# zju-pi/diff-sampler

Measured on AMD Instinct MI355X. Metric: images/sec (whole node) at NFE=10, EDM CIFAR-10, higher is better.
Workload: dtype fp32; 1 GPU; EDM CIFAR-10 32x32 SongUNet (55.7M params), DPM-Solver++(2M) logSNR NFE=10, batch 256/GPU; launch=eager

## Files before the change

### diff_sampler_amd/csrc/conv3x3_wino.hip

```cpp
#include <type_traits>

#include "igemm_common.h"

namespace igemm {
namespace {

typedef float f32x2 __attribute__((ext_vector_type(2)));

constexpr int WV_NO_NORM = 2, WV_NO_HALO = 4, WV_NO_DMA = 8, WV_NO_EPI = 16;
constexpr int WINO_K = 8;
constexpr int WINO_POS = 2 * 64 * 4;
constexpr int WINO_IMG = 16 * WINO_POS;
constexpr int WINO_NSH = 4;
constexpr int WINO_EPI_LD = 36;

#define DS_WINO_WAIT_VM0() do { __builtin_amdgcn_s_waitcnt(0x0F70); asm volatile("" ::: "memory"); } while (0)
#define DS_WINO_WAIT_VM(n) do { __builtin_amdgcn_s_waitcnt(0x0F70 | (n)); asm volatile("" ::: "memory"); } while (0)

template <int VAR, int NORM, int NSL>
__global__ void __launch_bounds__(256, 1) conv3x3_wino_kernel(const KParams p) {
    extern __shared__ __attribute__((aligned(16))) float smem[];
    float* Us = smem;
    float* Vs = smem + 2 * WINO_IMG;
    float* Hs = Vs + WINO_IMG;

    const int tid = threadIdx.x, lane = tid & 63;
    const int wave = __builtin_amdgcn_readfirstlane(tid >> 6);
    const int wr = wave >> 1, wc = wave & 1;
    int mt, nt;
    if (!decode_tile(blockIdx.x, p.mtiles, p.ntiles, mt, nt)) return;
    const int m0 = mt * 256, n0 = nt * 64;
    const int img0 = m0 / p.HW;
    const int r0 = (m0 - img0 * p.HW) / p.W;
    const int WPH = p.WP >> 1, Wt = p.W >> 1;
    const int Ctot = p.c0 + p.c1;
    const int nslabs = Ctot / WINO_K;
    constexpr bool kDma = !(VAR & WV_NO_DMA), kHalo = !(VAR & WV_NO_HALO);
    constexpr int kNorm = (VAR & WV_NO_NORM) ? 0 : NORM;

    const int kh_h = tid & 1;
    unsigned h_off0[WINO_NSH], h_off1[WINO_NSH];
    int h_lds[WINO_NSH];
    bool h_ok[WINO_NSH];
#pragma unroll
    for (int j = 0; j < WINO_NSH; ++j) {
        const int hp = (tid + j * 256) >> 1;
        const int hr = hp / p.WP, hc = hp - hr * p.WP;
        const int y = r0 + hr - 1, x = hc - 1;
        const bool in = hp < p.NP;
        h_ok[j] = in && (unsigned)y < (unsigned)p.H && (unsigned)x < (unsigned)p.W;
        const int pix = min(max(y, 0), p.H - 1) * p.W + min(max(x, 0), p.W - 1);
        h_off0[j] = (unsigned)(pix * p.lda0 + kh_h * 4);
        h_off1[j] = (unsigned)(pix * p.lda1 + kh_h * 4);
        h_lds[j] = in ? (((kh_h * 2 + (hc & 1)) * p.HP + hr) * WPH + (hc >> 1)) * 4 : p.NP * WINO_K;
    }
    const float* a0i = p.a0 + (size_t)img0 * p.HW * p.lda0;
    const float* a1i = p.a1 + (size_t)img0 * p.HW * p.lda1;
    const float* cpi = p.norm + (size_t)img0 * 3 * Ctot + kh_h * 4;
    f32x4 hreg[WINO_NSH];
    float h_t[4 * WINO_NSH], h_u[4 * WINO_NSH];
    f32x4 cmu = {0.f, 0.f, 0.f, 0.f}, cga = {1.f, 1.f, 1.f, 1.f}, cbe = {0.f, 0.f, 0.f, 0.f};
    const float* h_src = nullptr;
    unsigned h_sel = 0;
    auto halo_src = [&](int s) {
        const int c = s * WINO_K;
        const bool first = c < p.c0;
        h_src = first ? a0i + c : a1i + (c - p.c0);
        h_sel = (unsigned)__builtin_amdgcn_readfirstlane(first ? -1 : 0);
        asm volatile("" : "+s"(h_sel));
    };
    auto halo_load1 = [&](auto J) {
        constexpr int j = decltype(J)::value;
        if constexpr (j >= NSL) return;
        const unsigned off = (h_off0[j] & h_sel) | (h_off1[j] & ~h_sel);
        hreg[j] = *reinterpret_cast<const f32x4*>(h_src + off);
    };
    auto coef_load1 = [&](int s, auto I) {
        constexpr int i = decltype(I)::value;
        if constexpr (NORM != 0) {
            const f32x4 v = *reinterpret_cast<const f32x4*>(cpi + (size_t)i * Ctot + s * WINO_K);
            if constexpr (i == 0) cmu = v; else if constexpr (i == 1) cga = v; else cbe = v;
        }
    };
    auto halo_chain = [&](auto C, auto ST) {
        constexpr int c = decltype(C)::value, st = decltype(ST)::value, j = c >> 2, e = c & 3;
        if constexpr (j >= NSL) return;
        if constexpr (st == 0 && kNorm != 0) {
            h_t[c] = __builtin_fmaf(hreg[j][e] - cmu[e], cga[e], cbe[e]);
            if constexpr (kNorm == 2) h_u[c] = __expf(-h_t[c]);
        }
        if constexpr (st == 1 && kNorm == 2) h_u[c] = __builtin_amdgcn_rcpf(1.0f + h_u[c]);
        if constexpr (st == 2) {
            float v = hreg[j][e];
            if constexpr (kNorm == 1) v = h_t[c];
            if constexpr (kNorm == 2) v = h_t[c] * h_u[c];
            hreg[j][e] = h_ok[j] ? v : 0.f;
            if constexpr (e == 3) *reinterpret_cast<f32x4*>(Hs + h_lds[j]) = hreg[j];
        }
    };

    const int t_t = (tid >> 1) & 63, cpl = tid & 1, kh_t = tid >> 7;
    const int t_ty = t_t / Wt, t_tx = t_t - t_ty * Wt;
    const float* h_rd = Hs + ((kh_t * 2 * p.HP + 2 * t_ty) * WPH + t_tx) * 4 + cpl * 2;
    const int h_par = p.HP * WPH * 4;
    float* v_wr = Vs + (kh_t * 64 + t_t) * 4 + cpl * 2;
    auto transform = [&]() {
        f32x2 d[4][4];
#pragma unroll
        for (int i = 0; i < 4; ++i)
#pragma unroll
            for (int j = 0; j < 4; ++j)
                d[i][j] = *reinterpret_cast<const f32x2*>(h_rd + (j & 1) * h_par + i * WPH * 4 + (j >> 1) * 4);
        DS_RACE_SKEW(wave);
        f32x2 t[4][4];
#pragma unroll
        for (int j = 0; j < 4; ++j) {
            t[0][j] = d[0][j] - d[2][j];
            t[1][j] = d[1][j] + d[2][j];
            t[2][j] = d[2][j] - d[1][j];
            t[3][j] = d[1][j] - d[3][j];
        }
#pragma unroll
        for (int i = 0; i < 4; ++i) {
            *reinterpret_cast<f32x2*>(v_wr + (i * 4 + 0) * WINO_POS) = t[i][0] - t[i][2];
            *reinterpret_cast<f32x2*>(v_wr + (i * 4 + 1) * WINO_POS) = t[i][1] + t[i][2];
            *reinterpret_cast<f32x2*>(v_wr + (i * 4 + 2) * WINO_POS) = t[i][2] - t[i][1];
            *reinterpret_cast<f32x2*>(v_wr + (i * 4 + 3) * WINO_POS) = t[i][1] - t[i][3];
        }
    };

    const float* u_src = p.b + (size_t)nt * nslabs * WINO_IMG + tid * 4;
    auto u_dma1 = [&](const float* src, float* ubuf, auto I) {
        constexpr int i = decltype(I)::value;
        float* dst = ubuf + (i * 256 + wave * 64) * 4;
        typedef const __attribute__((address_space(1))) void* gptr_t;
        typedef __attribute__((address_space(3))) void* lptr_t;
        __builtin_amdgcn_global_load_lds((gptr_t)(src + i * 1024), (lptr_t)(dst), 16, 0, 0);
    };

    f32x16 acc[16];
#pragma unroll
    for (int q = 0; q < 16; ++q)
#pragma unroll
        for (int r = 0; r < 16; ++r) acc[q][r] = 0.f;
    const int a_off = ((lane >> 5) * 64 + wr * 32 + (lane & 31)) * 4;
    const int b_off = ((lane >> 5) * 64 + wc * 32 + (lane & 31)) * 4;

#define DS_WINO_I(n) std::integral_constant<int, (n)>{}
#define DS_WINO_EACH4(F) F(0) F(1) F(2) F(3)
#define DS_WINO_EACH16(F, b) F((b) + 0) F((b) + 1) F((b) + 2) F((b) + 3) F((b) + 4) F((b) + 5) F((b) + 6) F((b) + 7)                \
                             F((b) + 8) F((b) + 9) F((b) + 10) F((b) + 11) F((b) + 12) F((b) + 13) F((b) + 14) F((b) + 15)

    halo_src(0);
#define DS_WINO_F(j) halo_load1(DS_WINO_I(j));
    DS_WINO_EACH4(DS_WINO_F)
#undef DS_WINO_F
    coef_load1(0, DS_WINO_I(0)); coef_load1(0, DS_WINO_I(1)); coef_load1(0, DS_WINO_I(2));
    DS_RACE_SKEW(wave);
#define DS_WINO_F(i) u_dma1(u_src, Us, DS_WINO_I(i)); u_dma1(u_src, Us, DS_WINO_I((i) + 4));
    DS_WINO_EACH4(DS_WINO_F)
#undef DS_WINO_F
    DS_RACE_SKEW(wave);
#define DS_WINO_F(c) halo_chain(DS_WINO_I(c), DS_WINO_I(0)); halo_chain(DS_WINO_I(c), DS_WINO_I(1)); halo_chain(DS_WINO_I(c), DS_WINO_I(2));
    DS_WINO_EACH16(DS_WINO_F, 0)
#undef DS_WINO_F
    {
        const int s1 = min(1, nslabs - 1);
        halo_src(s1);
#define DS_WINO_F(j) halo_load1(DS_WINO_I(j));
        DS_WINO_EACH4(DS_WINO_F)
#undef DS_WINO_F
        coef_load1(s1, DS_WINO_I(0)); coef_load1(s1, DS_WINO_I(1)); coef_load1(s1, DS_WINO_I(2));
    }
    DS_WINO_WAIT_VM0();
    __syncthreads();

    f32x4 fa[2][4], fb[2][4];
    int s = 0;
    do {
        const float* ub = Us + (s & 1) * WINO_IMG;
        transform();
        __syncthreads();
        const int s1 = min(s + 1, nslabs - 1), s2 = min(s + 2, nslabs - 1);
        const float* un = u_src + (size_t)s1 * WINO_IMG;
        float* ubn = Us + ((s + 1) & 1) * WINO_IMG;
        if constexpr (kHalo) halo_src(s2);
        auto frag_read = [&](auto G, auto I) {
            constexpr int g = decltype(G)::value, i = decltype(I)::value;
            if constexpr (i < 4) fa[g & 1][i] = *reinterpret_cast<const f32x4*>(Vs + (g * 4 + i) * WINO_POS + a_off);
            else fb[g & 1][i - 4] = *reinterpret_cast<const f32x4*>(ub + (g * 4 + i - 4) * WINO_POS + b_off);
        };
        if constexpr (kHalo) {
            DS_RACE_SKEW(wave);
#define DS_WINO_F(c) halo_chain(DS_WINO_I(c), DS_WINO_I(0)); halo_chain(DS_WINO_I(c), DS_WINO_I(1)); halo_chain(DS_WINO_I(c), DS_WINO_I(2));
            DS_WINO_EACH16(DS_WINO_F, 0)
#undef DS_WINO_F
        }
        auto fill = [&](auto K) {
            constexpr int k = decltype(K)::value, g = k >> 4;
            if constexpr (k < 8) {
                if constexpr (kDma) {
                    if constexpr (k == 0) DS_RACE_SKEW(wave);
                    u_dma1(un, ubn, DS_WINO_I(k));
                }
            } else if constexpr (k < 12) {
                if constexpr (kHalo) halo_load1(DS_WINO_I(k - 8));
            } else if constexpr (k < 15) {
                if constexpr (kHalo) coef_load1(s2, DS_WINO_I(k - 12));
            }
            constexpr int fr = g == 0 ? 8 : g == 1 ? 20 : g == 2 ? 32 : 64;
            if constexpr (k >= fr && k < fr + 8) frag_read(DS_WINO_I(g + 1), DS_WINO_I(k - fr));
        };
#define DS_WINO_STEP(k)                                                                                                                \
        acc[((k) >> 4) * 4 + ((k) & 3)] = __builtin_amdgcn_mfma_f32_32x32x2f32(fa[((k) >> 4) & 1][(k) & 3][((k) >> 2) & 3],            \
                                                                               fb[((k) >> 4) & 1][(k) & 3][((k) >> 2) & 3],            \
                                                                               acc[((k) >> 4) * 4 + ((k) & 3)], 0, 0, 0);              \
        fill(DS_WINO_I(k));                                                                                                            \
        __builtin_amdgcn_sched_barrier(0);
#define DS_WINO_F(i) frag_read(DS_WINO_I(0), DS_WINO_I(i)); frag_read(DS_WINO_I(0), DS_WINO_I((i) + 4));
        DS_WINO_EACH4(DS_WINO_F)
#undef DS_WINO_F
        __builtin_amdgcn_sched_barrier(0);
        DS_WINO_EACH16(DS_WINO_STEP, 0)
        DS_WINO_EACH16(DS_WINO_STEP, 16)
        DS_WINO_EACH16(DS_WINO_STEP, 32)
        DS_WINO_EACH16(DS_WINO_STEP, 48)
#undef DS_WINO_STEP
        DS_WINO_WAIT_VM0();
        __syncthreads();
    } while (++s < nslabs);

    if constexpr ((VAR & WV_NO_EPI) != 0) {
#pragma unroll
        for (int q = 0; q < 16; ++q) asm volatile("" :: "v"(acc[q]));
        return;
    }

    f32x16 Y[4];
#pragma unroll
    for (int a = 0; a < 2; ++a) {
        f32x16 t[4];
#pragma unroll
        for (int j = 0; j < 4; ++j) t[j] = a == 0 ? acc[j] + acc[4 + j] + acc[8 + j] : acc[4 + j] - acc[8 + j] - acc[12 + j];
        Y[a * 2 + 0] = t[0] + t[1] + t[2];
        Y[a * 2 + 1] = t[1] - t[2] - t[3];
    }

    const int nextra = (p.ec0 + p.ec1) / 32;
    if (nextra > 0) {
        const float* wsk = p.b + (size_t)p.ntiles * nslabs * WINO_IMG + (size_t)nt * nextra * 2048 + tid * 4;
        const int e_chunk = tid & 7;
        int e_lds[8];
#pragma unroll
        for (int j = 0; j < 8; ++j) {
            const int lp = (tid >> 3) + 32 * j;
            const int yl = lp / p.W, x = lp - yl * p.W;
            const int ph = (yl & 1) * 2 + (x & 1), t = (yl >> 1) * Wt + (x >> 1);
            e_lds[j] = (((ph * 4 + (e_chunk >> 1)) * 2 + (e_chunk & 1)) * 64 + (t ^ e_chunk)) * 4;
        }
        int ea_off[4];
#pragma unroll
        for (int g = 0; g < 4; ++g) ea_off[g] = ((lane >> 5) * 64 + ((wr * 32 + (lane & 31)) ^ (2 * g + (lane >> 5)))) * 4;
        const unsigned e_t0 = (unsigned)((tid >> 3) * p.elda0 + e_chunk * 4), e_t1 = (unsigned)((tid >> 3) * p.elda1 + e_chunk * 4);
        const float* e_src = nullptr;
        unsigned e_off = 0;
        int e_step = 0;
        auto e_sel = [&](int es) {
            const int c = es * 32;
            const bool first = c < p.ec0;
            const int ld = first ? p.elda0 : p.elda1;
            e_src = (first ? p.e0 + c : p.e1 + (c - p.ec0)) + (size_t)m0 * ld;
            e_step = 32 * ld;
            e_off = first ? e_t0 : e_t1;
        };
        auto e_load1 = [&](f32x4* dst, auto J) {
            constexpr int j = decltype(J)::value;
            dst[j] = *reinterpret_cast<const f32x4*>(e_src + (size_t)(j * e_step) + e_off);
        };
        auto w_dma1 = [&](int es, float* wbuf, auto I) {
            constexpr int i = decltype(I)::value;
            float* dst = wbuf + (i * 256 + wave * 64) * 4;
            typedef const __attribute__((address_space(1))) void* gptr_t;
            typedef __attribute__((address_space(3))) void* lptr_t;
            __builtin_amdgcn_global_load_lds((gptr_t)(wsk + (size_t)es * 2048 + i * 1024), (lptr_t)(dst), 16, 0, 0);
        };
#define DS_WINO_EACH8(F) F(0) F(1) F(2) F(3) F(4) F(5) F(6) F(7)

        f32x4 ereg[8];
        {
            f32x4 ereg0[8];
            DS_RACE_SKEW(wave);
            w_dma1(0, smem, DS_WINO_I(0)); w_dma1(0, smem, DS_WINO_I(1));
            e_sel(0);
#define DS_WINO_F(j) e_load1(ereg0, DS_WINO_I(j));
            DS_WINO_EACH8(DS_WINO_F)
#undef DS_WINO_F
            e_sel(min(1, nextra - 1));
#define DS_WINO_F(j) e_load1(ereg, DS_WINO_I(j));
            DS_WINO_EACH8(DS_WINO_F)
#undef DS_WINO_F
            DS_WINO_WAIT_VM(8);
            DS_RACE_SKEW(wave);
#pragma unroll
            for (int j = 0; j < 8; ++j) *reinterpret_cast<f32x4*>(Vs + e_lds[j]) = ereg0[j];
        }
        __syncthreads();

        f32x4 ga[2][4], gb[2];
        int es = 0;
        do {
            const float* vb = smem + (2 - (es & 1)) * WINO_IMG;
            float* vn = smem + (1 + (es & 1)) * WINO_IMG;
            const float* wb = smem + (es & 1) * 2048;
            float* wn = smem + ((es + 1) & 1) * 2048;
            const int es1 = min(es + 1, nextra - 1);
            e_sel(min(es + 2, nextra - 1));
            auto frag_read = [&](auto G, auto I) {
                constexpr int g = decltype(G)::value, i = decltype(I)::value;
                if constexpr (i < 4) ga[g & 1][i] = *reinterpret_cast<const f32x4*>(vb + (i * 4 + g) * WINO_POS + ea_off[g]);
                else gb[g & 1] = *reinterpret_cast<const f32x4*>(wb + g * WINO_POS + b_off);
            };
            auto fill = [&](auto K) {
                constexpr int k = decltype(K)::value, g = k >> 4;
                if constexpr (k < 2) {
                    if constexpr (k == 0) DS_RACE_SKEW(wave);
                    w_dma1(es1, wn, DS_WINO_I(k));
                } else if constexpr (k >= 7 && k < 15) {
                    if constexpr (k == 7) DS_RACE_SKEW(wave);
                    *reinterpret_cast<f32x4*>(vn + e_lds[k - 7]) = ereg[k - 7];
                } else if constexpr (k >= 15 && k < 23) {
                    e_load1(ereg, DS_WINO_I(k - 15));
                }
                constexpr int fr = g == 0 ? 2 : g == 1 ? 24 : g == 2 ? 36 : 64;
                if constexpr (k >= fr && k < fr + 5) frag_read(DS_WINO_I(g + 1), DS_WINO_I(k - fr));
            };
#define DS_WINO_STEP(k)                                                                                                                \
            Y[(k) & 3] = __builtin_amdgcn_mfma_f32_32x32x2f32(ga[((k) >> 4) & 1][(k) & 3][((k) >> 2) & 3], gb[((k) >> 4) & 1][((k) >> 2) & 3], \
                                                              Y[(k) & 3], 0, 0, 0);                                                    \
            fill(DS_WINO_I(k));                                                                                                        \
            __builtin_amdgcn_sched_barrier(0);
            frag_read(DS_WINO_I(0), DS_WINO_I(0)); frag_read(DS_WINO_I(0), DS_WINO_I(4)); frag_read(DS_WINO_I(0), DS_WINO_I(1));
            frag_read(DS_WINO_I(0), DS_WINO_I(2)); frag_read(DS_WINO_I(0), DS_WINO_I(3));
            __builtin_amdgcn_sched_barrier(0);
            DS_WINO_EACH16(DS_WINO_STEP, 0)
            DS_WINO_EACH16(DS_WINO_STEP, 16)
            DS_WINO_EACH16(DS_WINO_STEP, 32)
            DS_WINO_EACH16(DS_WINO_STEP, 48)
#undef DS_WINO_STEP
            DS_WINO_WAIT_VM0();
            __syncthreads();
        } while (++es < nextra);
#undef DS_WINO_EACH8
    }
#undef DS_WINO_EACH16
#undef DS_WINO_EACH4
#undef DS_WINO_I

    float* stage = smem + wave * 32 * WINO_EPI_LD;
    const int c4 = (lane & 7) * 4;
    const int col = n0 + wc * 32 + c4;
    f32x4 cb = {0.f, 0.f, 0.f, 0.f}, cvu = {0.f, 0.f, 0.f, 0.f};
    if (p.colbias) cb = *reinterpret_cast<const f32x4*>(p.colbias + col);
    if (p.cbias) cvu = *reinterpret_cast<const f32x4*>(p.cbias + (size_t)(p.cbias_bcast ? 0 : img0) * p.cbias_ld + col);
    const float acc_scale = __builtin_bit_cast(float, __builtin_amdgcn_readfirstlane(__builtin_bit_cast(int, p.acc_scale)));
    const float scale = __builtin_bit_cast(float, __builtin_amdgcn_readfirstlane(__builtin_bit_cast(int, p.scale)));
    int e_row[4];
#pragma unroll
    for (int pass = 0; pass < 4; ++pass) {
        const int tl = wr * 32 + pass * 8 + (lane >> 3);
        const int ty = tl / Wt, tx = tl - ty * Wt;
        e_row[pass] = m0 + 2 * ty * p.W + 2 * tx;
    }
#pragma unroll
    for (int a = 0; a < 2; ++a) {
        f32x4 st_s = {0.f, 0.f, 0.f, 0.f}, st_q = {0.f, 0.f, 0.f, 0.f};
#pragma unroll
        for (int b = 0; b < 2; ++b) {
            const f32x16 y = Y[a * 2 + b];
            f32x4 rv[4];
            if (p.res) {
#pragma unroll
                for (int pass = 0; pass < 4; ++pass)
                    rv[pass] = __builtin_nontemporal_load(reinterpret_cast<const f32x4*>(p.res + (size_t)(e_row[pass] + a * p.W + b) * p.res_ld + col));
            }
#pragma unroll
            for (int r = 0; r < 16; ++r) stage[((r & 3) + 8 * (r >> 2) + 4 * (lane >> 5)) * WINO_EPI_LD + (lane & 31)] = y[r];
#pragma unroll
            for (int pass = 0; pass < 4; ++pass) {
                f32x4 v = *reinterpret_cast<const f32x4*>(stage + (pass * 8 + (lane >> 3)) * WINO_EPI_LD + c4);
                v *= acc_scale;
                v += cb;
                if (p.cbias) v += cvu;
                if (p.res) v += rv[pass];
                v *= scale;
                if (p.act == DS_ACT_SILU) {
#pragma unroll
                    for (int q = 0; q < 4; ++q) v[q] = ds_silu(v[q]);
                }
                __builtin_nontemporal_store(v, reinterpret_cast<f32x4*>(p.out + (size_t)(e_row[pass] + a * p.W + b) * p.ldo + col));
                st_s += v; st_q += v * v;
            }
        }
        if (p.stats) {
#pragma unroll
            for (int q = 0; q < 4; ++q) {
                st_s[q] += __shfl_xor(st_s[q], 8); st_s[q] += __shfl_xor(st_s[q], 16); st_s[q] += __shfl_xor(st_s[q], 32);
                st_q[q] += __shfl_xor(st_q[q], 8); st_q[q] += __shfl_xor(st_q[q], 16); st_q[q] += __shfl_xor(st_q[q], 32);
            }
            if (lane < 8) {
                float* sp = p.stats + (size_t)((m0 >> 6) + wr * 2 + a) * 2 * p.N + col;
                *reinterpret_cast<f32x4*>(sp) = st_s;
                *reinterpret_cast<f32x4*>(sp + p.N) = st_q;
            }
        }
    }
}

template <int VAR, int NORM, int NSL>
int launch_wino_ns(KParams& p, hipStream_t stream) {
    const int smem = (3 * WINO_IMG + p.NP * WINO_K + 4) * (int)sizeof(float);
    DS_ENSURE_DYN_LDS((&conv3x3_wino_kernel<VAR, NORM, NSL>), 128 * 1024);
    hipLaunchKernelGGL((conv3x3_wino_kernel<VAR, NORM, NSL>), dim3(grid_1d(p.mtiles, p.ntiles)), dim3(256), smem, stream, p);
    DS_CHECK_LAUNCH();
    return DS_OK;
}

template <int VAR, int NORM>
int launch_wino_n(KParams& p, hipStream_t stream) {
    return p.NP * 2 <= 3 * 256 ? launch_wino_ns<VAR, NORM, 3>(p, stream) : launch_wino_ns<VAR, NORM, 4>(p, stream);
}

template <int VAR>
int launch_wino(KParams& p, hipStream_t stream) {
    if (!p.norm) return launch_wino_n<VAR, 0>(p, stream);
    return p.norm_act == DS_ACT_SILU ? launch_wino_n<VAR, 2>(p, stream) : launch_wino_n<VAR, 1>(p, stream);
}

}

bool conv3x3_wino_applicable(const KParams& p) {
    if (p.taps != 9 || p.stride != 1 || p.splits != 1 || (p.ec0 & 31) || (p.ec1 & 31)) return false;
    if ((p.H & 1) || (p.W & 1) || p.W < 4 || p.W > 64 || p.HW % 256 || 256 % p.W || ((256 / p.W) & 1)) return false;
    if ((p.N & 63) || (p.c0 % WINO_K) || (p.c1 % WINO_K) || !p.vec_ok || p.out_planar || p.out_f16 || p.res_f16 || p.rowbias) return false;
    if (p.act != DS_ACT_NONE && p.act != DS_ACT_SILU) return false;
    const int np = (256 / p.W + 2) * (p.W + 2);
    if (np * 2 > WINO_NSH * 256 || (3 * WINO_IMG + np * WINO_K + 4) * (int)sizeof(float) > 128 * 1024) return false;
    return p.M % 256 == 0;
}

int launch_conv3x3_wino(KParams& p, hipStream_t stream) {
    if (!conv3x3_wino_applicable(p)) return DS_E_SHAPE;
    p.TH = 256 / p.W; p.nimg = 1; p.HP = p.TH + 2; p.WP = p.W + 2; p.NP = p.HP * p.WP;
    p.mtiles = p.M / 256; p.ntiles = p.N / 64; p.n_begin = 0;
#ifdef DS_CONV_ABLATIONS
    if (p.t_variant & 0x10000) {
        switch (p.t_variant & 31) {
            case 2: return launch_wino<2>(p, stream);
            case 4: return launch_wino<4>(p, stream);
            case 8: return launch_wino<8>(p, stream);
            case 16: return launch_wino<16>(p, stream);
            case 28: return launch_wino<28>(p, stream);
            default: break;
        }
    }
#endif
    return launch_wino<0>(p, stream);
}

}
```

Before: 446.3 images/sec.

## Double-buffer Winograd V and halo LDS to drop per-slab barrier

Restructures the Winograd 3x3 conv main loop so the input transform for slab s+1 is computed into a second V buffer while the GEMM consumes slab s. The halo staging area is double-buffered, and halo loads are prefetched three slabs ahead using two register sets. This removes the mid-iteration __syncthreads and transform stall between transform and MMA. The cost is raising the LDS footprint to up to 160 KB, plus byte-offset address tricks meant to keep global loads in SGPR-base plus VGPR-offset form.

Result: faster. 463.6 images/sec (median of 6 runs) (+3.9%).

```diff
diff --git a/diff_sampler_amd/csrc/conv3x3_wino.hip b/diff_sampler_amd/csrc/conv3x3_wino.hip
--- a/diff_sampler_amd/csrc/conv3x3_wino.hip
+++ b/diff_sampler_amd/csrc/conv3x3_wino.hip
@@ -22,7 +22,7 @@
     extern __shared__ __attribute__((aligned(16))) float smem[];
     float* Us = smem;
     float* Vs = smem + 2 * WINO_IMG;
-    float* Hs = Vs + WINO_IMG;
+    float* Hs = smem + 4 * WINO_IMG;
 
     const int tid = threadIdx.x, lane = tid & 63;
     const int wave = __builtin_amdgcn_readfirstlane(tid >> 6);
@@ -50,16 +50,21 @@
         const bool in = hp < p.NP;
         h_ok[j] = in && (unsigned)y < (unsigned)p.H && (unsigned)x < (unsigned)p.W;
         const int pix = min(max(y, 0), p.H - 1) * p.W + min(max(x, 0), p.W - 1);
-        h_off0[j] = (unsigned)(pix * p.lda0 + kh_h * 4);
-        h_off1[j] = (unsigned)(pix * p.lda1 + kh_h * 4);
+        h_off0[j] = (unsigned)(pix * p.lda0 + kh_h * 4) * 4u;
+        h_off1[j] = (unsigned)(pix * p.lda1 + kh_h * 4) * 4u;
         h_lds[j] = in ? (((kh_h * 2 + (hc & 1)) * p.HP + hr) * WPH + (hc >> 1)) * 4 : p.NP * WINO_K;
     }
     const float* a0i = p.a0 + (size_t)img0 * p.HW * p.lda0;
     const float* a1i = p.a1 + (size_t)img0 * p.HW * p.lda1;
-    const float* cpi = p.norm + (size_t)img0 * 3 * Ctot + kh_h * 4;
-    f32x4 hreg[WINO_NSH];
+    const float* cpi = p.norm + (size_t)img0 * 3 * Ctot;
+    unsigned c_lane = (unsigned)(kh_h * 16);
+    const int h_buf = p.NP * WINO_K + 4;
+    struct HaloRegs {
+        f32x4 h[WINO_NSH];
+        f32x4 mu = {0.f, 0.f, 0.f, 0.f}, ga = {1.f, 1.f, 1.f, 1.f}, be = {0.f, 0.f, 0.f, 0.f};
+    };
+    HaloRegs hreg;
     float h_t[4 * WINO_NSH], h_u[4 * WINO_NSH];
-    f32x4 cmu = {0.f, 0.f, 0.f, 0.f}, cga = {1.f, 1.f, 1.f, 1.f}, cbe = {0.f, 0.f, 0.f, 0.f};
     const float* h_src = nullptr;
     unsigned h_sel = 0;
     auto halo_src = [&](int s) {
@@ -69,73 +74,70 @@
         h_sel = (unsigned)__builtin_amdgcn_readfirstlane(first ? -1 : 0);
         asm volatile("" : "+s"(h_sel));
     };
-    auto halo_load1 = [&](auto J) {
+    auto halo_load1 = [&](HaloRegs& R, auto J) {
         constexpr int j = decltype(J)::value;
         if constexpr (j >= NSL) return;
         const unsigned off = (h_off0[j] & h_sel) | (h_off1[j] & ~h_sel);
-        hreg[j] = *reinterpret_cast<const f32x4*>(h_src + off);
-    };
-    auto coef_load1 = [&](int s, auto I) {
+        R.h[j] = *reinterpret_cast<const f32x4*>(reinterpret_cast<const char*>(h_src) + off);
+    };
+    auto coef_load1 = [&](HaloRegs& R, int s, auto I) {
         constexpr int i = decltype(I)::value;
         if constexpr (NORM != 0) {
-            const f32x4 v = *reinterpret_cast<const f32x4*>(cpi + (size_t)i * Ctot + s * WINO_K);
-            if constexpr (i == 0) cmu = v; else if constexpr (i == 1) cga = v; else cbe = v;
-        }
-    };
-    auto halo_chain = [&](auto C, auto ST) {
+            const char* cs = reinterpret_cast<const char*>(cpi + (size_t)i * Ctot + s * WINO_K);
+            asm volatile("" : "+v"(c_lane));
+            const f32x4 v = *reinterpret_cast<const f32x4*>(cs + c_lane);
+            if constexpr (i == 0) R.mu = v; else if constexpr (i == 1) R.ga = v; else R.be = v;
+        }
+    };
+    auto halo_chain = [&](HaloRegs& R, float* hs, auto C, auto ST) {
         constexpr int c = decltype(C)::value, st = decltype(ST)::value, j = c >> 2, e = c & 3;
         if constexpr (j >= NSL) return;
         if constexpr (st == 0 && kNorm != 0) {
-            h_t[c] = __builtin_fmaf(hreg[j][e] - cmu[e], cga[e], cbe[e]);
+            h_t[c] = __builtin_fmaf(R.h[j][e] - R.mu[e], R.ga[e], R.be[e]);
             if constexpr (kNorm == 2) h_u[c] = __expf(-h_t[c]);
         }
         if constexpr (st == 1 && kNorm == 2) h_u[c] = __builtin_amdgcn_rcpf(1.0f + h_u[c]);
         if constexpr (st == 2) {
-            float v = hreg[j][e];
+            float v = R.h[j][e];
             if constexpr (kNorm == 1) v = h_t[c];
             if constexpr (kNorm == 2) v = h_t[c] * h_u[c];
-            hreg[j][e] = h_ok[j] ? v : 0.f;
-            if constexpr (e == 3) *reinterpret_cast<f32x4*>(Hs + h_lds[j]) = hreg[j];
+            R.h[j][e] = h_ok[j] ? v : 0.f;
+            if constexpr (e == 3) *reinterpret_cast<f32x4*>(hs + h_lds[j]) = R.h[j];
         }
     };
 
     const int t_t = (tid >> 1) & 63, cpl = tid & 1, kh_t = tid >> 7;
     const int t_ty = t_t / Wt, t_tx = t_t - t_ty * Wt;
-    const float* h_rd = Hs + ((kh_t * 2 * p.HP + 2 * t_ty) * WPH + t_tx) * 4 + cpl * 2;
+    const int h_rd = ((kh_t * 2 * p.HP + 2 * t_ty) * WPH + t_tx) * 4 + cpl * 2;
     const int h_par = p.HP * WPH * 4;
-    float* v_wr = Vs + (kh_t * 64 + t_t) * 4 + cpl * 2;
-    auto transform = [&]() {
-        f32x2 d[4][4];
-#pragma unroll
-        for (int i = 0; i < 4; ++i)
-#pragma unroll
-            for (int j = 0; j < 4; ++j)
-                d[i][j] = *reinterpret_cast<const f32x2*>(h_rd + (j & 1) * h_par + i * WPH * 4 + (j >> 1) * 4);
-        DS_RACE_SKEW(wave);
-        f32x2 t[4][4];
-#pragma unroll
-        for (int j = 0; j < 4; ++j) {
-            t[0][j] = d[0][j] - d[2][j];
-            t[1][j] = d[1][j] + d[2][j];
-            t[2][j] = d[2][j] - d[1][j];
-            t[3][j] = d[1][j] - d[3][j];
-        }
-#pragma unroll
-        for (int i = 0; i < 4; ++i) {
-            *reinterpret_cast<f32x2*>(v_wr + (i * 4 + 0) * WINO_POS) = t[i][0] - t[i][2];
-            *reinterpret_cast<f32x2*>(v_wr + (i * 4 + 1) * WINO_POS) = t[i][1] + t[i][2];
-            *reinterpret_cast<f32x2*>(v_wr + (i * 4 + 2) * WINO_POS) = t[i][2] - t[i][1];
-            *reinterpret_cast<f32x2*>(v_wr + (i * 4 + 3) * WINO_POS) = t[i][1] - t[i][3];
-        }
-    };
-
-    const float* u_src = p.b + (size_t)nt * nslabs * WINO_IMG + tid * 4;
+    const int v_wr = (kh_t * 64 + t_t) * 4 + cpl * 2;
+    f32x2 t_d[4][4], t_r[4];
+    auto tr_read1 = [&](const float* hs, auto I) {
+        constexpr int i = decltype(I)::value >> 2, j = decltype(I)::value & 3;
+        t_d[i][j] = *reinterpret_cast<const f32x2*>(hs + h_rd + (j & 1) * h_par + i * WPH * 4 + (j >> 1) * 4);
+    };
+    auto tr_write1 = [&](float* vs, auto I) {
+        constexpr int i = decltype(I)::value >> 2, j = decltype(I)::value & 3;
+        if constexpr (j == 0) {
+#pragma unroll
+            for (int q = 0; q < 4; ++q)
+                t_r[q] = i == 0 ? t_d[0][q] - t_d[2][q] : i == 1 ? t_d[1][q] + t_d[2][q] : i == 2 ? t_d[2][q] - t_d[1][q] : t_d[1][q] - t_d[3][q];
+        }
+        const f32x2 v = j == 0 ? t_r[0] - t_r[2] : j == 1 ? t_r[1] + t_r[2] : j == 2 ? t_r[2] - t_r[1] : t_r[1] - t_r[3];
+        *reinterpret_cast<f32x2*>(vs + v_wr + (i * 4 + j) * WINO_POS) = v;
+    };
+
+    const float* u_src = p.b + (size_t)nt * nslabs * WINO_IMG;
+    unsigned u_lane = (unsigned)tid * 16u;
     auto u_dma1 = [&](const float* src, float* ubuf, auto I) {
         constexpr int i = decltype(I)::value;
         float* dst = ubuf + (i * 256 + wave * 64) * 4;
         typedef const __attribute__((address_space(1))) void* gptr_t;
         typedef __attribute__((address_space(3))) void* lptr_t;
-        __builtin_amdgcn_global_load_lds((gptr_t)(src + i * 1024), (lptr_t)(dst), 16, 0, 0);
+        const char* us = reinterpret_cast<const char*>(src + i * 1024);
+        asm volatile("" : "+s"(us));
+        asm volatile("" : "+v"(u_lane));
+        __builtin_amdgcn_global_load_lds((gptr_t)(us + u_lane), (lptr_t)(dst), 16, 0, 0);
     };
 
     f32x16 acc[16];
@@ -151,51 +153,80 @@
 #define DS_WINO_EACH16(F, b) F((b) + 0) F((b) + 1) F((b) + 2) F((b) + 3) F((b) + 4) F((b) + 5) F((b) + 6) F((b) + 7)                \
                              F((b) + 8) F((b) + 9) F((b) + 10) F((b) + 11) F((b) + 12) F((b) + 13) F((b) + 14) F((b) + 15)
 
+#define DS_WINO_LOADS(R, sl)                                                                                                           \
+    halo_load1(R, DS_WINO_I(0)); halo_load1(R, DS_WINO_I(1)); halo_load1(R, DS_WINO_I(2)); halo_load1(R, DS_WINO_I(3));                \
+    coef_load1(R, sl, DS_WINO_I(0)); coef_load1(R, sl, DS_WINO_I(1)); coef_load1(R, sl, DS_WINO_I(2));
+
     halo_src(0);
-#define DS_WINO_F(j) halo_load1(DS_WINO_I(j));
-    DS_WINO_EACH4(DS_WINO_F)
-#undef DS_WINO_F
-    coef_load1(0, DS_WINO_I(0)); coef_load1(0, DS_WINO_I(1)); coef_load1(0, DS_WINO_I(2));
-    DS_RACE_SKEW(wave);
-#define DS_WINO_F(i) u_dma1(u_src, Us, DS_WINO_I(i)); u_dma1(u_src, Us, DS_WINO_I((i) + 4));
-    DS_WINO_EACH4(DS_WINO_F)
-#undef DS_WINO_F
-    DS_RACE_SKEW(wave);
-#define DS_WINO_F(c) halo_chain(DS_WINO_I(c), DS_WINO_I(0)); halo_chain(DS_WINO_I(c), DS_WINO_I(1)); halo_chain(DS_WINO_I(c), DS_WINO_I(2));
-    DS_WINO_EACH16(DS_WINO_F, 0)
-#undef DS_WINO_F
+    DS_WINO_LOADS(hreg, 0)
     {
+        HaloRegs hreg1;
         const int s1 = min(1, nslabs - 1);
         halo_src(s1);
-#define DS_WINO_F(j) halo_load1(DS_WINO_I(j));
+        DS_WINO_LOADS(hreg1, s1)
+        DS_RACE_SKEW(wave);
+#define DS_WINO_F(i) u_dma1(u_src, Us, DS_WINO_I(i)); u_dma1(u_src, Us, DS_WINO_I((i) + 4));
         DS_WINO_EACH4(DS_WINO_F)
 #undef DS_WINO_F
-        coef_load1(s1, DS_WINO_I(0)); coef_load1(s1, DS_WINO_I(1)); coef_load1(s1, DS_WINO_I(2));
-    }
+        DS_RACE_SKEW(wave);
+#define DS_WINO_CHAIN1(c) halo_chain(hreg, Hs, DS_WINO_I(c), DS_WINO_I(0)); halo_chain(hreg, Hs, DS_WINO_I(c), DS_WINO_I(1));          \
+                          halo_chain(hreg, Hs, DS_WINO_I(c), DS_WINO_I(2));
+        DS_WINO_EACH16(DS_WINO_CHAIN1, 0)
+#undef DS_WINO_CHAIN1
+        DS_RACE_SKEW(wave);
+#define DS_WINO_CHAIN1(c) halo_chain(hreg1, Hs + h_buf, DS_WINO_I(c), DS_WINO_I(0)); halo_chain(hreg1, Hs + h_buf, DS_WINO_I(c), DS_WINO_I(1)); \
+                          halo_chain(hreg1, Hs + h_buf, DS_WINO_I(c), DS_WINO_I(2));
+        DS_WINO_EACH16(DS_WINO_CHAIN1, 0)
+#undef DS_WINO_CHAIN1
+    }
+    {
+        const int s2 = min(2, nslabs - 1);
+        halo_src(s2);
+        DS_WINO_LOADS(hreg, s2)
+    }
+    __syncthreads();
+#define DS_WINO_F(i) tr_read1(Hs, DS_WINO_I(i));
+    DS_WINO_EACH16(DS_WINO_F, 0)
+#undef DS_WINO_F
+    DS_RACE_SKEW(wave);
+#define DS_WINO_F(i) tr_write1(Vs, DS_WINO_I(i));
+    DS_WINO_EACH16(DS_WINO_F, 0)
+#undef DS_WINO_F
     DS_WINO_WAIT_VM0();
     __syncthreads();
 
     f32x4 fa[2][4], fb[2][4];
     int s = 0;
     do {
-        const float* ub = Us + (s & 1) * WINO_IMG;
-        transform();
-        __syncthreads();
-        const int s1 = min(s + 1, nslabs - 1), s2 = min(s + 2, nslabs - 1);
+        const int par = s & 1;
+        const float* ub = Us + par * WINO_IMG;
+        const float* vb = Vs + par * WINO_IMG;
+        float* ubn = Us + (par ^ 1) * WINO_IMG;
+        float* vbn = Vs + (par ^ 1) * WINO_IMG;
+        float* hb = Hs + par * h_buf;
+        const float* hbn = Hs + (par ^ 1) * h_buf;
+        const int s1 = min(s + 1, nslabs - 1), s3 = min(s + 3, nslabs - 1);
         const float* un = u_src + (size_t)s1 * WINO_IMG;
-        float* ubn = Us + ((s + 1) & 1) * WINO_IMG;
-        if constexpr (kHalo) halo_src(s2);
         auto frag_read = [&](auto G, auto I) {
             constexpr int g = decltype(G)::value, i = decltype(I)::value;
-            if constexpr (i < 4) fa[g & 1][i] = *reinterpret_cast<const f32x4*>(Vs + (g * 4 + i) * WINO_POS + a_off);
+            if constexpr (i < 4) fa[g & 1][i] = *reinterpret_cast<const f32x4*>(vb + (g * 4 + i) * WINO_POS + a_off);
             else fb[g & 1][i - 4] = *reinterpret_cast<const f32x4*>(ub + (g * 4 + i - 4) * WINO_POS + b_off);
         };
+#define DS_WINO_F(i) tr_read1(hbn, DS_WINO_I(i));
+        DS_WINO_EACH16(DS_WINO_F, 0)
+#undef DS_WINO_F
         if constexpr (kHalo) {
             DS_RACE_SKEW(wave);
-#define DS_WINO_F(c) halo_chain(DS_WINO_I(c), DS_WINO_I(0)); halo_chain(DS_WINO_I(c), DS_WINO_I(1)); halo_chain(DS_WINO_I(c), DS_WINO_I(2));
-            DS_WINO_EACH16(DS_WINO_F, 0)
-#undef DS_WINO_F
-        }
+#define DS_WINO_CHAIN1(c) halo_chain(hreg, hb, DS_WINO_I(c), DS_WINO_I(0)); halo_chain(hreg, hb, DS_WINO_I(c), DS_WINO_I(1));          \
+                          halo_chain(hreg, hb, DS_WINO_I(c), DS_WINO_I(2));
+            DS_WINO_EACH16(DS_WINO_CHAIN1, 0)
+#undef DS_WINO_CHAIN1
+            halo_src(s3);
+        }
+        DS_RACE_SKEW(wave);
+#define DS_WINO_F(i) tr_write1(vbn, DS_WINO_I(i));
+        DS_WINO_EACH16(DS_WINO_F, 0)
+#undef DS_WINO_F
         auto fill = [&](auto K) {
             constexpr int k = decltype(K)::value, g = k >> 4;
             if constexpr (k < 8) {
@@ -204,9 +235,9 @@
                     u_dma1(un, ubn, DS_WINO_I(k));
                 }
             } else if constexpr (k < 12) {
-                if constexpr (kHalo) halo_load1(DS_WINO_I(k - 8));
+                if constexpr (kHalo) halo_load1(hreg, DS_WINO_I(k - 8));
             } else if constexpr (k < 15) {
-                if constexpr (kHalo) coef_load1(s2, DS_WINO_I(k - 12));
+                if constexpr (kHalo) coef_load1(hreg, s3, DS_WINO_I(k - 12));
             }
             constexpr int fr = g == 0 ? 8 : g == 1 ? 20 : g == 2 ? 32 : 64;
             if constexpr (k >= fr && k < fr + 8) frag_read(DS_WINO_I(g + 1), DS_WINO_I(k - fr));
@@ -229,6 +260,7 @@
         DS_WINO_WAIT_VM0();
         __syncthreads();
     } while (++s < nslabs);
+#undef DS_WINO_LOADS
 
     if constexpr ((VAR & WV_NO_EPI) != 0) {
 #pragma unroll
@@ -418,8 +450,8 @@
 
 template <int VAR, int NORM, int NSL>
 int launch_wino_ns(KParams& p, hipStream_t stream) {
-    const int smem = (3 * WINO_IMG + p.NP * WINO_K + 4) * (int)sizeof(float);
-    DS_ENSURE_DYN_LDS((&conv3x3_wino_kernel<VAR, NORM, NSL>), 128 * 1024);
+    const int smem = (4 * WINO_IMG + 2 * (p.NP * WINO_K + 4)) * (int)sizeof(float);
+    DS_ENSURE_DYN_LDS((&conv3x3_wino_kernel<VAR, NORM, NSL>), 160 * 1024);
     hipLaunchKernelGGL((conv3x3_wino_kernel<VAR, NORM, NSL>), dim3(grid_1d(p.mtiles, p.ntiles)), dim3(256), smem, stream, p);
     DS_CHECK_LAUNCH();
     return DS_OK;
@@ -444,7 +476,7 @@
     if ((p.N & 63) || (p.c0 % WINO_K) || (p.c1 % WINO_K) || !p.vec_ok || p.out_planar || p.out_f16 || p.res_f16 || p.rowbias) return false;
     if (p.act != DS_ACT_NONE && p.act != DS_ACT_SILU) return false;
     const int np = (256 / p.W + 2) * (p.W + 2);
-    if (np * 2 > WINO_NSH * 256 || (3 * WINO_IMG + np * WINO_K + 4) * (int)sizeof(float) > 128 * 1024) return false;
+    if (np * 2 > WINO_NSH * 256 || (4 * WINO_IMG + 2 * (np * WINO_K + 4)) * (int)sizeof(float) > 160 * 1024) return false;
     return p.M % 256 == 0;
 }
 
```
